# Alexander-H-Liu/End-to-end-ASR-Pytorch

Hardware: NVIDIA H100
Metric: utterances/sec (train step, ~12s@16kHz synthetic) (higher is better)
Workload: dtype f32

## Files before the change

### end-to-end-asr-pytorch_b200/csrc/lstm.cu

```cuda
#include "common.cuh"
#include "lstm_umma.h"
#include "../../include/b200asr.h"
#include "../../include/b200asr_debug.h"

namespace b200asr {

constexpr int LSTM_GTHREADS = 128;
constexpr int LSTM_THREADS = 2 * LSTM_GTHREADS + 64;
constexpr int LSTM_NCHUNK = 4;
constexpr int LSTM_MAX_TILES = 32;
constexpr int LSTM_CHUNK_PAD = 4;
constexpr int LSTM_COUNTER_BYTES = 4096;

struct LstmParams {
    float* gates;
    const float* whh;
    float* cst;
    float* out;
    float* xbuf;
    unsigned* counters;
    int* err_flag;
    int B, T, H, ndir, UB, Bc, nub, nbg, NH, R;
    int b0, Bend;
    int mma;
// ... 1320 lines not shown
extern "C" int b200asr_bilstm_plan(int B, int H, int ndir, int* unit_block, int* batch_block, int* n_ctas) {
    Plan pl;
    const int rc = make_plan(B, H, ndir, &pl);
    B200_REQUIRE(rc == 0, "bilstm_plan: no feasible decomposition for B=%d H=%d ndir=%d (H must be a multiple of 16)",
                 B, H, ndir);
    if (unit_block) *unit_block = pl.UB;
    if (batch_block) *batch_block = pl.Bc;
    if (n_ctas) *n_ctas = pl.ctas;
    return B200_OK;
}

extern "C" int b200asr_bilstm_uses_tensor_cores(int B, int H, int ndir) {
    Plan pl;
    if (make_plan(B, H, ndir, &pl) != 0) return -1;
    return pl.mma ? 1 : 0;
}

static int bilstm_run(bool bwd, float* gates, const float* w_hh, float* cstate, float* out_or_dout, int B, int T,
                      int H, int ndir, void* workspace, size_t workspace_bytes, cudaStream_t stream) {
    B200_REQUIRE(gates && w_hh && cstate && out_or_dout && workspace, "bilstm: null pointer");
    B200_REQUIRE(B > 0 && T > 0 && H > 0 && (ndir == 1 || ndir == 2), "bilstm: bad sizes B=%d T=%d H=%d ndir=%d", B, T,
                 H, ndir);
    Plan pl;
    LstmVariant v;
    B200_REQUIRE(lstm_variant(B, H, ndir, bwd, &pl, &v) == 0,
                 "bilstm: no feasible decomposition for B=%d H=%d ndir=%d (H must be a multiple of 16)", B, H, ndir);
    B200_REQUIRE(workspace_bytes >= b200asr_bilstm_workspace_bytes(B, T, H, ndir), "bilstm: workspace too small");
    if (v.gen == 1 && !bwd)
        return lstm_umma_fwd(gates, w_hh, cstate, out_or_dout, B, T, H, ndir, workspace, workspace_bytes, v.strict != 0,
                             stream);
    if (v.gen == 1)
        return lstm_umma_bwd(gates, w_hh, cstate, out_or_dout, B, T, H, ndir, workspace, workspace_bytes, stream);
    unsigned char* ws = reinterpret_cast<unsigned char*>(workspace);
    float* packed = reinterpret_cast<float*>(ws);
    const size_t xoff = align_up(pl.pack_bytes, 256);
    const size_t xbytes = pl.xbuf_fwd_bytes > pl.xbuf_bwd_bytes ? pl.xbuf_fwd_bytes : pl.xbuf_bwd_bytes;
    float* xbuf = reinterpret_cast<float*>(ws + xoff);
    unsigned* counters = reinterpret_cast<unsigned*>(ws + xoff + align_up(xbytes, 256));
    int* err_flag = reinterpret_cast<int*>(counters + (LSTM_COUNTER_BYTES / 4 - 4));

    {
        const long long n = (long long)(pl.pack_bytes / sizeof(float));
        int blocks = (int)((n + 255) / 256);
        if (blocks > 4096) blocks = 4096;
        if (pl.mma) lstm_pack_mma_kernel<<<blocks, 256, 0, stream>>>(w_hh, packed, H, pl.UB, ndir, bwd ? 1 : 0);
        else lstm_pack_kernel<<<blocks, 256, 0, stream>>>(w_hh, packed, H, pl.UB, ndir, bwd ? 1 : 0);
        B200_LAUNCH_CHECK("lstm_pack_kernel");
    }
    LstmParams p;
    p.gates = gates; p.whh = packed; p.cst = cstate; p.out = out_or_dout; p.xbuf = xbuf; p.counters = counters;
    p.err_flag = err_flag; p.B = B; p.T = T; p.H = H; p.ndir = ndir; p.UB = pl.UB; p.Bc = pl.Bc; p.nub = pl.nub;
    p.nbg = pl.nbg; p.NH = pl.NH; p.R = pl.R; p.mma = pl.mma; p.form = v.form;
    const void* fn = !pl.mma ? (bwd ? (const void*)bilstm_bwd_kernel : (const void*)bilstm_fwd_kernel)
                             : (bwd ? (const void*)bilstm_bwd_mma_kernel : (const void*)bilstm_fwd_mma_kernel);
    const size_t smem = bwd ? pl.smem_bwd : pl.smem_fwd;
    B200_REQUIRE(smem <= (size_t)max_optin_smem(), "bilstm: %zu B of shared memory exceed the device limit", smem);
    B200_CUDA(cudaFuncSetAttribute(fn, cudaFuncAttributeMaxDynamicSharedMemorySize, (int)smem));
    int per_sm = 0;
    B200_CUDA(cudaOccupancyMaxActiveBlocksPerMultiprocessor(&per_sm, fn, LSTM_THREADS, smem));
    B200_REQUIRE((long long)per_sm * sm_count() >= pl.ctas, "bilstm: %d CTAs cannot be co-resident (%d/SM x %d SMs)",
                 pl.ctas, per_sm, sm_count());
    for (int sp = 0; sp < pl.nsplit; ++sp) {
        p.b0 = sp * pl.Bsub;
        p.Bend = p.b0 + pl.Bsub < B ? p.b0 + pl.Bsub : B;
        B200_CUDA(cudaMemsetAsync(counters, 0, LSTM_COUNTER_BYTES, stream));
        void* args[] = {&p};
        B200_CUDA(cudaLaunchCooperativeKernel(fn, dim3(pl.ctas), dim3(LSTM_THREADS), args, smem, stream));
        count_launch();
    }
    return B200_OK;
}

extern "C" int b200asr_debug_lstm_variant(int B, int H, int ndir, int bwd, int* desc) {
    Plan pl;
    LstmVariant v;
    if (B <= 0 || H <= 0 || (ndir != 1 && ndir != 2) || !desc) return -1;
    const int rc = lstm_variant(B, H, ndir, bwd != 0, &pl, &v);
    if (rc != 0) return rc;
    const int d[9] = {v.gen, v.UB, v.UBP, v.poll, v.strict, v.nsplit, v.form, v.R, v.vec};
    for (int i = 0; i < 9; ++i) desc[i] = d[i];
    return 0;
}

extern "C" void b200asr_debug_set_lstm_mode(int mode) {
    g_lstm_mode = mode & 3;
    g_lstm_strict = (mode & 256) != 0;
}

extern "C" int b200asr_bilstm_fwd(float* gates, const float* w_hh, float* cstate, float* out, int B, int T, int H,
                                  int ndir, void* workspace, size_t workspace_bytes, b200asr_stream stream) {
    return bilstm_run(false, gates, w_hh, cstate, out, B, T, H, ndir, workspace, workspace_bytes,
                      (cudaStream_t)stream);
}

extern "C" int b200asr_bilstm_bwd(float* gates, const float* w_hh, const float* cstate, const float* dout, int B,
                                  int T, int H, int ndir, void* workspace, size_t workspace_bytes,
                                  b200asr_stream stream) {
    return bilstm_run(true, gates, w_hh, const_cast<float*>(cstate), const_cast<float*>(dout), B, T, H, ndir,
                      workspace, workspace_bytes, (cudaStream_t)stream);
}

extern "C" int b200asr_lstm_cell_fwd(const float* preact, const float* c_prev, float* gates, float* c, float* h,
                                     int B, int H, b200asr_stream stream) {
    B200_REQUIRE(preact && c_prev && gates && c && h, "lstm_cell_fwd: null pointer");
    B200_REQUIRE(B > 0 && H > 0, "lstm_cell_fwd: bad sizes");
    const int n = B * H;
    lstm_cell_fwd_kernel<<<(n + 255) / 256, 256, 0, (cudaStream_t)stream>>>(preact, c_prev, gates, c, h, B, H);
    B200_LAUNCH_CHECK("lstm_cell_fwd_kernel");
    return B200_OK;
}

extern "C" int b200asr_lstm_cell_bwd(const float* gates, const float* c_prev, const float* c, const float* dh,
                                     const float* dc_next, float* dpreact, float* dc_prev, int B, int H,
                                     b200asr_stream stream) {
    B200_REQUIRE(gates && c_prev && c && dh && dpreact && dc_prev, "lstm_cell_bwd: null pointer");
    B200_REQUIRE(B > 0 && H > 0, "lstm_cell_bwd: bad sizes");
    const int n = B * H;
    lstm_cell_bwd_kernel<<<(n + 255) / 256, 256, 0, (cudaStream_t)stream>>>(gates, c_prev, c, dh, dc_next, dpreact,
                                                                          dc_prev, B, H);
    B200_LAUNCH_CHECK("lstm_cell_bwd_kernel");
    return B200_OK;
}
```

### end-to-end-asr-pytorch_b200/csrc/lstm_umma.cu

```cuda
#include <cuda_fp16.h>
#include "common.cuh"
#include "wgmma.cuh"
#include "lstm_umma.h"

namespace b200asr {
namespace {

constexpr int UL_BC = 32;
constexpr int UL_MAX_CTRL = 8;
constexpr int UL_ATOM_A = 64 * 128;
constexpr int UL_MAX_ATOMS = 16;
constexpr int UL_COUNTER_BYTES = 4096;

struct UlParams {
    float* gates;
    const uint8_t* wpack;
    float* cst;
    float* out;
    uint8_t* xbuf;
    unsigned* counters;
    int* err_flag;
    int B, T, H, ndir, UB, nub, nbg, NA, NC;
    int strict;
    int b0, Bend;
// ... 183 lines not shown
                if (st_pending) {
                    *reinterpret_cast<float4*>(p.gates + (st_row * H + ug) * 4) = st_g;
                    p.cst[st_row * H + ug] = st_c;
                    p.out[st_out] = st_h;
                    st_pending = false;
                }
                const float k = 1.f / 2048.f;
                pre.x += dif[0] + (dif[2] + eif[0]) * k;
                pre.y += dif[1] + (dif[3] + eif[1]) * k;
                pre.z += dgo[0] + (dgo[2] + ego[0]) * k;
                pre.w += dgo[1] + (dgo[3] + ego[1]) * k;
            }
            const float ig = sigmoidf_(pre.x);
            const float fg = sigmoidf_(pre.y);
            const float gg = tanhf(pre.z);
            const float og = sigmoidf_(pre.w);
            const float c = fmaf(fg, c_reg, ig * gg);
            c_reg = ok ? c : 0.f;
            const float hq = ok ? og * tanhf(c) : 0.f;
            if (step + 1 < T) {
                uint8_t* dstimg = xb + (size_t)(step & 1) * img_bytes;
                __half hi, lo;
                split_f16(hq, hi, lo);
                if ((UB & 3) == 0) {
                    uint32_t wh = __half_as_ushort(hi), wl = __half_as_ushort(lo);
                    wh |= __shfl_down_sync(0xffffffffu, wh, 1) << 16;
                    wl |= __shfl_down_sync(0xffffffffu, wl, 1) << 16;
                    const uint32_t wh2 = __shfl_down_sync(0xffffffffu, wh, 2);
                    const uint32_t wl2 = __shfl_down_sync(0xffffffffu, wl, 2);
                    if (tq == 0 && unit < UB) {
                        *reinterpret_cast<uint2*>(dstimg + pub_hi) = make_uint2(wh, wh2);
                        *reinterpret_cast<uint2*>(dstimg + pub_lo) = make_uint2(wl, wl2);
                    }
                } else if (unit < UB) {
                    *reinterpret_cast<__half*>(dstimg + pub_hi) = hi;
                    *reinterpret_cast<__half*>(dstimg + pub_lo) = lo;
                }
                __syncwarp();
                if (lane == 0) ul_arrive(pub);
            }
            st_g = make_float4(ig, fg, gg, og);
            st_c = c;
            st_h = hq;
            st_row = rowbase;
            st_out = ((size_t)brow * T + tt) * (p.ndir * H) + (size_t)dir * H + ug;
            st_pending = ok;
        }
        if (st_pending) {
            *reinterpret_cast<float4*>(p.gates + (st_row * H + ug) * 4) = st_g;
            p.cst[st_row * H + ug] = st_c;
            p.out[st_out] = st_h;
        }
    }
}

template <int UB>
__global__ void ul_pack_bwd_kernel(const float* __restrict__ w, uint8_t* __restrict__ dst, int H, int ndir) {
    const int nub = H / UB;
    const long long per_cta = (long long)2 * H * 64;
    const long long n_el = (long long)ndir * nub * per_cta;
    for (long long i = (long long)blockIdx.x * blockDim.x + threadIdx.x; i < n_el; i += (long long)gridDim.x * blockDim.x) {
        const int cta = (int)(i / per_cta);
        int r = (int)(i - (long long)cta * per_cta);
        const int part = r / (H * 64);
        r -= part * H * 64;
        const int n = r >> 6, k = r & 63;
        const int dir = cta / nub, ub = cta - dir * nub;
        const int u = k >> 2, g = k & 3;
        float v = 0.f;
        if (u < UB) v = w[((long long)dir * 4 * H + (long long)g * H + (ub * UB + u)) * H + n];
        __half hi, lo;
        split_f16(v, hi, lo);
        uint8_t* img = dst + (size_t)cta * ((size_t)2 * H * 128) + (size_t)part * H * 128;
        *reinterpret_cast<__half*>(img + wgmma::sw128_offset(n, k * 2)) = part ? lo : hi;
    }
}


__device__ __forceinline__ float add_ftz(float a, float b) {
    float r;
    asm("add.ftz.f32 %0, %1, %2;" : "=f"(r) : "f"(a), "f"(b));
    return r;
}

constexpr int ULB_EPI_WARPS = 16;
constexpr int ULB_CTRL = 4;

template <int UB>
__global__ void __launch_bounds__(32 * (ULB_EPI_WARPS + 1 + ULB_CTRL), 1) bilstm_bwd_umma_kernel(UlParams p) {
    constexpr int KS = (4 * UB) / 16;
    extern __shared__ __align__(1024) uint8_t smem[];
    const int H = p.H, T = p.T, nub = p.nub;
    const int NB = (H + 255) / 256;
    uint8_t* sWhi = smem;
    uint8_t* sWlo = smem + (size_t)H * 128;
    uint8_t* sA1 = sWlo + (size_t)H * 128;
    uint8_t* sA2 = sA1 + 8192;
    float* rscale = reinterpret_cast<float*>(sA2 + 8192);
    uint64_t* a_ready = reinterpret_cast<uint64_t*>(rscale + 32);
    uint64_t* mma_done = a_ready + 1;
    uint64_t* wload = a_ready + 2;

    const int tid = threadIdx.x, warp = tid >> 5, lane = tid & 31;
    int blk = blockIdx.x;
    const int ub = blk % p.nub; blk /= p.nub;
    const int bg = blk % p.nbg; blk /= p.nbg;
    const int dir = blk;

    for (int i = tid; i < 16384 / 16; i += blockDim.x) reinterpret_cast<uint4*>(sA1)[i] = make_uint4(0, 0, 0, 0);
    if (tid == 0) {
        mbar_init(a_ready, ULB_EPI_WARPS);
        mbar_init(mma_done, ULB_EPI_WARPS);
        mbar_init(wload, 1);
        mbar_fence_init();
    }
    fence_proxy_async_smem();
    __syncthreads();
    const size_t xelems = (size_t)nub * nub * UL_BC * UB;
    float* xb = reinterpret_cast<float*>(p.xbuf) + ((size_t)dir * p.nbg + bg) * 2 * xelems;

    if (warp >= ULB_EPI_WARPS) {
        if (warp == ULB_EPI_WARPS + 1 && lane == 0) {
            const uint8_t* wsrc = p.wpack + ((size_t)dir * p.nub + ub) * ((size_t)2 * H * 128);
            mbar_expect_tx(wload, (uint32_t)(2 * H * 128));
            for (int off = 0; off < 2 * H * 128; off += 32768)
                bulk_g2s(sWhi + off, wsrc + off, 32768, wload);
        }
    } else {
        const int ci = warp * 32 + lane;
        const bool cell = ci < UL_BC * UB;
        const int b = cell ? ci / UB : 0, u = cell ? ci % UB : 0;
        const int brow = p.b0 + bg * UL_BC + b;
        const bool ok = cell && brow < p.Bend;
        const int ug = ub * UB + u;
        const int row_hi = 16 * (b >> 3) + (b & 7), row_lo = row_hi + 8;
        const uint32_t off_hi = wgmma::sw128_offset(row_hi, 8 * u), off_lo = wgmma::sw128_offset(row_lo, 8 * u);
        const int q = warp & 3, jq = warp >> 2, r = lane >> 2, tq = lane & 3;
        const int drow = 8 * q + r;
        const uint32_t a1 = smem_u32(sA1), a2 = smem_u32(sA2), whi = smem_u32(sWhi), wlo = smem_u32(sWlo);
        float d[32];
        float dc_reg = 0.f;

        for (int step = 0; step < T; ++step) {
            const int fstep = T - 1 - step;
            const int tt = dir ? (T - 1 - fstep) : fstep;
            const int tt_prev = dir ? tt + 1 : tt - 1;
            float4 gtv = make_float4(0.f, 0.f, 0.f, 0.f);
            float ct = 0.f, cp = 0.f, dh = 0.f;
            const size_t row = ((size_t)dir * p.B + (ok ? brow : 0)) * T + tt;
            if (ok) {
                gtv = *reinterpret_cast<const float4*>(p.gates + (row * H + ug) * 4);
                ct = p.cst[row * H + ug];
                if (fstep > 0) cp = p.cst[(((size_t)dir * p.B + brow) * T + tt_prev) * H + ug];
                dh = p.out[((size_t)brow * T + tt) * (p.ndir * H) + (size_t)dir * H + ug];
            }
            if (step > 0) {
                if (cell) {
                    const float* ib = xb + (size_t)((step - 1) & 1) * xelems + (size_t)ub * nub * UL_BC * UB +
                                      (size_t)b * UB + u;
                    const uint32_t tag = (uint32_t)(((step - 1) >> 1) & 1) ^ 1u;
                    const long long t0 = clock64();
                    float s0 = 0.f, s1 = 0.f, s2 = 0.f, s3 = 0.f;
                    for (int sb = 0; sb < nub; sb += 32) {
                        float v[32];
                        const int nhere = min(32, nub - sb);
                        v[0] = ld_relaxed_f32(ib + (size_t)sb * UL_BC * UB);
                        while ((__float_as_uint(v[0]) & 1u) != tag) {
                            ul_watchdog(t0, p.err_flag);
                            v[0] = ld_relaxed_f32(ib + (size_t)sb * UL_BC * UB);
                        }
#pragma unroll
                        for (int j = 1; j < 32; ++j)
                            v[j] = (j < nhere) ? ld_relaxed_f32(ib + (size_t)(sb + j) * UL_BC * UB) : __uint_as_float(tag);
                        uint32_t pending = 0;
#pragma unroll
                        for (int j = 1; j < 32; ++j) pending |= ((__float_as_uint(v[j]) & 1u) != tag) ? (1u << j) : 0u;
                        while (pending) {
                            ul_watchdog(t0, p.err_flag);
#pragma unroll
                            for (int j = 1; j < 32; ++j)
                                if (pending & (1u << j)) {
                                    v[j] = ld_relaxed_f32(ib + (size_t)(sb + j) * UL_BC * UB);
                                    if ((__float_as_uint(v[j]) & 1u) == tag) pending &= ~(1u << j);
                                }
                        }
#pragma unroll
                        for (int j = 0; j < 32; j += 4) {
                            if (j < nhere) {
                                s0 = add_ftz(s0, v[j]); s1 = add_ftz(s1, v[j + 1]);
                                s2 = add_ftz(s2, v[j + 2]); s3 = add_ftz(s3, v[j + 3]);
                            }
                        }
                    }
                    dh += (s0 + s1) + (s2 + s3);
                }
            }
            float4 dg = make_float4(0.f, 0.f, 0.f, 0.f);
            if (ok) {
                const float ig = gtv.x, fg = gtv.y, gg = gtv.z, og = gtv.w;
                const float tc = tanhf(ct);
                const float dc = dc_reg + dh * og * (1.f - tc * tc);
                dg.x = dc * gg * ig * (1.f - ig);
                dg.y = dc * cp * fg * (1.f - fg);
                dg.z = dc * ig * (1.f - gg * gg);
                dg.w = dh * tc * og * (1.f - og);
                dc_reg = dc * fg;
                *reinterpret_cast<float4*>(p.gates + (row * H + ug) * 4) = dg;
            }
            if (step + 1 < T) {
                float m = fmaxf(fmaxf(fabsf(dg.x), fabsf(dg.y)), fmaxf(fabsf(dg.z), fabsf(dg.w)));
#pragma unroll
                for (int o = 1; o < UB; o <<= 1) m = fmaxf(m, __shfl_xor_sync(0xffffffffu, m, o));
                int e = (int)((__float_as_uint(m) >> 23) & 0xffu) - 127;
                e = e < -113 ? -113 : (e > 127 ? 127 : e);
                const float sc = __uint_as_float((uint32_t)(127 + 13 - e) << 23);
                if (step > 0) mbar_wait(mma_done, (uint32_t)((step - 1) & 1));
                if (cell) {
                    if (u == 0) rscale[b] = __uint_as_float((uint32_t)(127 + e - 13) << 23);
                    __half hi[4], lo[4];
                    split_f16(dg.x * sc, hi[0], lo[0]);
                    split_f16(dg.y * sc, hi[1], lo[1]);
                    split_f16(dg.z * sc, hi[2], lo[2]);
                    split_f16(dg.w * sc, hi[3], lo[3]);
                    const uint2 vh = make_uint2((uint32_t)__half_as_ushort(hi[0]) | ((uint32_t)__half_as_ushort(hi[1]) << 16),
                                                (uint32_t)__half_as_ushort(hi[2]) | ((uint32_t)__half_as_ushort(hi[3]) << 16));
                    const uint2 vl = make_uint2((uint32_t)__half_as_ushort(lo[0]) | ((uint32_t)__half_as_ushort(lo[1]) << 16),
                                                (uint32_t)__half_as_ushort(lo[2]) | ((uint32_t)__half_as_ushort(lo[3]) << 16));
                    *reinterpret_cast<uint2*>(sA1 + off_hi) = vh;
                    *reinterpret_cast<uint2*>(sA1 + off_lo) = vl;
                    *reinterpret_cast<uint2*>(sA2 + off_lo) = vh;
                }
                fence_proxy_async_smem();
                __syncwarp();
                if (lane == 0) ul_arrive(a_ready);
                if (step == 0) mbar_wait(wload, 0);
                mbar_wait(a_ready, (uint32_t)(step & 1));
                float* outbase = xb + (size_t)(step & 1) * xelems;
                for (int j = 0; j < NB; ++j) {
                    if (256 * j + 64 * jq >= H) continue;
                    const uint32_t boff = (uint32_t)(256 * j + 64 * jq) * 128u;
                    wgmma::fence_operand(d);
                    wgmma::fence();
#pragma unroll
                    for (int kk = 0; kk < KS; ++kk) {
                        wgmma::mma_f16_n64(d, wgmma::desc_k_sw128(a1 + kk * 32), wgmma::desc_k_sw128(whi + boff + kk * 32), kk > 0);
                        wgmma::mma_f16_n64(d, wgmma::desc_k_sw128(a2 + kk * 32), wgmma::desc_k_sw128(wlo + boff + kk * 32), 1);
                    }
                    wgmma::commit_group();
                    wgmma::wait_all();
                    wgmma::fence_operand(d);
                    const float* v0 = d;
                    const float* v1 = d + 16;
                    const float rs = rscale[drow];
                    const float k = 1.f / 2048.f;
#pragma unroll
                    for (int hh = 0; hh < 2; ++hh) {
#pragma unroll
                        for (int g = 0; g < 4; ++g) {
                            const float* v = hh ? &v1[4 * g] : &v0[4 * g];
                            const int n = 256 * j + 64 * jq + 32 * hh + 8 * g + 2 * tq;
                            const int dst = n / UB, uu = n - dst * UB;
                            const float o0 = (v[0] + v[2] * k) * rs;
                            const float o1 = (v[1] + v[3] * k) * rs;
                            float* optr = outbase + (((size_t)dst * nub + ub) * UL_BC + drow) * UB + uu;
                            const uint32_t tagw = (uint32_t)((step >> 1) & 1) ^ 1u;
                            st_relaxed_v2(optr, (__float_as_uint(o0) & ~1u) | tagw, (__float_as_uint(o1) & ~1u) | tagw);
                        }
                    }
                }
                __syncwarp();
                if (lane == 0) ul_arrive(mma_done);
            }
        }
    }
}

struct UlPlan {
    int UB, UBp, nub, nbg, ctas, NA, Bsub, nsplit;
    size_t smem, pack_bytes, xbuf_bytes;
};

int ul_plan(int B, int H, int ndir, UlPlan* out) {
    if (H % 64 != 0 || H / 64 > UL_MAX_ATOMS) return -1;
    const int sms = sm_count();
    const size_t cap = (size_t)max_optin_smem();
    const int NA = H / 64;
    for (int n = 1; n <= B; ++n) {
        const int Bs = (B + n - 1) / n;
        const int nbg = (Bs + UL_BC - 1) / UL_BC;
        for (int UB = 2; UB <= 16; ++UB) {
            if (H % UB) continue;
            const int UBp = (UB + 3) / 4 * 4;
            if (UBp != 8 && UBp != 12 && UBp != 16) continue;
            const int nub = H / UB;
            const int ctas = ndir * nbg * nub;
            if (ctas > sms) continue;
            const size_t smem = (size_t)NA * UL_ATOM_A + (size_t)NA * 8 * UBp * 128 + 512;
            if (smem > cap) continue;
            if ((size_t)ndir * nbg * UL_MAX_ATOMS * 4 > UL_COUNTER_BYTES - 64) continue;
            out->UB = UB; out->UBp = UBp; out->nub = nub; out->nbg = nbg; out->ctas = ctas; out->NA = NA;
            out->Bsub = Bs; out->nsplit = (B + Bs - 1) / Bs; out->smem = smem;
            out->pack_bytes = (size_t)ndir * nub * NA * 8 * UBp * 128;
            out->xbuf_bytes = (size_t)ndir * nbg * 2 * NA * UL_ATOM_A;
            return 0;
        }
        if (Bs <= UL_BC) break;
    }
    return -2;
}

size_t ul_align(size_t x) { return (x + 255) / 256 * 256; }

template <int UBP>
int ul_launch_fwd(const UlPlan& pl, UlParams p, const float* w_hh, cudaStream_t stream) {
    {
        const long long n = (long long)p.ndir * pl.nub * 8 * UBP * p.H;
        int blocks = (int)((n + 255) / 256);
        if (blocks > 8192) blocks = 8192;
        ul_pack_fwd_kernel<UBP><<<blocks, 256, 0, stream>>>(w_hh, const_cast<uint8_t*>(p.wpack), p.H, pl.UB, p.ndir);
        B200_LAUNCH_CHECK("ul_pack_fwd_kernel");
    }
    const void* fn = (const void*)bilstm_fwd_umma_kernel<UBP>;
    B200_CUDA(cudaFuncSetAttribute(fn, cudaFuncAttributeMaxDynamicSharedMemorySize, (int)pl.smem));
    int per_sm = 0;
    const int threads = 32 * (UBP + 1 + p.NC);
    B200_CUDA(cudaOccupancyMaxActiveBlocksPerMultiprocessor(&per_sm, fn, threads, pl.smem));
    B200_REQUIRE((long long)per_sm * sm_count() >= pl.ctas, "bilstm(umma): %d CTAs cannot be co-resident (%d/SM x %d SMs)",
                 pl.ctas, per_sm, sm_count());
    for (int sp = 0; sp < pl.nsplit; ++sp) {
        p.b0 = sp * pl.Bsub;
        p.Bend = p.b0 + pl.Bsub < p.B ? p.b0 + pl.Bsub : p.B;
        B200_CUDA(cudaMemsetAsync(p.counters, 0, UL_COUNTER_BYTES, stream));
        void* args[] = {&p};
        B200_CUDA(cudaLaunchCooperativeKernel(fn, dim3(pl.ctas), dim3(threads), args, pl.smem, stream));
        count_launch();
    }
    return B200_OK;
}

struct UlbPlan {
    int UB, nub, nbg, ctas, Bsub, nsplit;
    size_t smem, pack_bytes, xbuf_bytes;
};

int ulb_plan(int B, int H, int ndir, UlbPlan* out) {
    if (H % 128 != 0 || H < 256 || H > 768) return -1;
    const int sms = sm_count();
    const size_t cap = (size_t)max_optin_smem();
    for (int n = 1; n <= B; ++n) {
        const int Bs = (B + n - 1) / n;
        const int nbg = (Bs + UL_BC - 1) / UL_BC;
        for (int UB = 8; UB <= 16; UB += 8) {
            if (H % UB) continue;
            const int nub = H / UB;
            const int ctas = ndir * nbg * nub;
            if (ctas > sms) continue;
            if (nub % 4) continue;
            const size_t inbox = (size_t)nub * UL_BC * UB * 4;
            const size_t smem = (size_t)2 * H * 128 + 16384 + 128 + 128;
            if (smem > cap || (inbox / ULB_CTRL) % 16 || (2 * H * 128) % 32768) continue;
            out->UB = UB; out->nub = nub; out->nbg = nbg; out->ctas = ctas; out->Bsub = Bs;
            out->nsplit = (B + Bs - 1) / Bs; out->smem = smem;
            out->pack_bytes = (size_t)ndir * nub * 2 * H * 128;
            out->xbuf_bytes = (size_t)ndir * nbg * 2 * nub * inbox;
            return 0;
        }
        if (Bs <= UL_BC) break;
    }
    return -2;
}

template <int UB>
int ul_launch_bwd(const UlbPlan& pl, UlParams p, const float* w_hh, cudaStream_t stream) {
    {
        const long long n = (long long)p.ndir * pl.nub * 2 * p.H * 64;
        int blocks = (int)((n + 255) / 256);
        if (blocks > 8192) blocks = 8192;
        ul_pack_bwd_kernel<UB><<<blocks, 256, 0, stream>>>(w_hh, const_cast<uint8_t*>(p.wpack), p.H, p.ndir);
        B200_LAUNCH_CHECK("ul_pack_bwd_kernel");
    }
    const void* fn = (const void*)bilstm_bwd_umma_kernel<UB>;
    B200_CUDA(cudaFuncSetAttribute(fn, cudaFuncAttributeMaxDynamicSharedMemorySize, (int)pl.smem));
    int per_sm = 0;
    const int threads = 32 * (ULB_EPI_WARPS + 1 + ULB_CTRL);
    B200_CUDA(cudaOccupancyMaxActiveBlocksPerMultiprocessor(&per_sm, fn, threads, pl.smem));
    B200_REQUIRE((long long)per_sm * sm_count() >= pl.ctas, "bilstm(umma bwd): %d CTAs cannot be co-resident (%d/SM x %d SMs)",
                 pl.ctas, per_sm, sm_count());
    for (int sp = 0; sp < pl.nsplit; ++sp) {
        p.b0 = sp * pl.Bsub;
        p.Bend = p.b0 + pl.Bsub < p.B ? p.b0 + pl.Bsub : p.B;
        B200_CUDA(cudaMemsetAsync(p.counters, 0, UL_COUNTER_BYTES, stream));
        B200_CUDA(cudaMemsetAsync(p.xbuf, 0, pl.xbuf_bytes, stream));
        void* args[] = {&p};
        B200_CUDA(cudaLaunchCooperativeKernel(fn, dim3(pl.ctas), dim3(threads), args, pl.smem, stream));
        count_launch();
    }
    return B200_OK;
}

}

bool lstm_umma_bwd_variant(int B, int H, int ndir, int* ub, int* nsplit) {
    UlbPlan pl;
    if (ulb_plan(B, H, ndir, &pl) != 0) return false;
    *ub = pl.UB;
    *nsplit = pl.nsplit;
    return true;
}

bool lstm_umma_fwd_variant(int B, int H, int ndir, int* ub, int* ubp, int* nsplit) {
    UlPlan pl;
    if (ul_plan(B, H, ndir, &pl) != 0) return false;
    *ub = pl.UB;
    *ubp = pl.UBp;
    *nsplit = pl.nsplit;
    return true;
}

int lstm_umma_bwd(float* gates, const float* w_hh, const float* cstate, const float* dout, int B, int T, int H, int ndir,
                  void* workspace, size_t workspace_bytes, cudaStream_t stream) {
    UlbPlan pl;
    B200_REQUIRE(ulb_plan(B, H, ndir, &pl) == 0, "bilstm(umma bwd): unsupported shape B=%d H=%d ndir=%d", B, H, ndir);
    B200_REQUIRE(workspace_bytes >= lstm_umma_workspace_bytes(B, H, ndir), "bilstm(umma bwd): workspace too small");
    uint8_t* ws = reinterpret_cast<uint8_t*>(workspace);
    UlParams p;
    p.gates = gates; p.cst = const_cast<float*>(cstate); p.out = const_cast<float*>(dout);
    p.wpack = ws;
    p.xbuf = ws + ul_align(pl.pack_bytes);
    p.counters = reinterpret_cast<unsigned*>(ws + ul_align(pl.pack_bytes) + ul_align(pl.xbuf_bytes));
    p.err_flag = reinterpret_cast<int*>(p.counters + (UL_COUNTER_BYTES / 4 - 4));
    p.B = B; p.T = T; p.H = H; p.ndir = ndir; p.UB = pl.UB; p.nub = pl.nub; p.nbg = pl.nbg; p.NA = 0; p.NC = ULB_CTRL;
    p.strict = 0;
    p.b0 = 0; p.Bend = B;
    if (pl.UB == 16) return ul_launch_bwd<16>(pl, p, w_hh, stream);
    return ul_launch_bwd<8>(pl, p, w_hh, stream);
}

size_t lstm_umma_workspace_bytes(int B, int H, int ndir) {
    UlPlan pl;
    UlbPlan pb;
    size_t f = 0, b = 0;
    if (ul_plan(B, H, ndir, &pl) == 0) f = ul_align(pl.pack_bytes) + ul_align(pl.xbuf_bytes) + UL_COUNTER_BYTES;
    if (ulb_plan(B, H, ndir, &pb) == 0) b = ul_align(pb.pack_bytes) + ul_align(pb.xbuf_bytes) + UL_COUNTER_BYTES;
    return f > b ? f : b;
}

int lstm_umma_plan(int B, int H, int ndir, int* unit_block, int* batch_block, int* n_ctas) {
    UlPlan pl;
    if (ul_plan(B, H, ndir, &pl) != 0) return -1;
    if (unit_block) *unit_block = pl.UB;
    if (batch_block) *batch_block = UL_BC;
    if (n_ctas) *n_ctas = pl.ctas;
    return 0;
}

int lstm_umma_fwd(float* gates, const float* w_hh, float* cstate, float* out, int B, int T, int H, int ndir,
                  void* workspace, size_t workspace_bytes, bool strict, cudaStream_t stream) {
    UlPlan pl;
    B200_REQUIRE(ul_plan(B, H, ndir, &pl) == 0, "bilstm(umma): unsupported shape B=%d H=%d ndir=%d", B, H, ndir);
    B200_REQUIRE(workspace_bytes >= lstm_umma_workspace_bytes(B, H, ndir), "bilstm(umma): workspace too small");
    uint8_t* ws = reinterpret_cast<uint8_t*>(workspace);
    UlParams p;
    p.gates = gates; p.cst = cstate; p.out = out;
    p.wpack = ws;
    p.xbuf = ws + ul_align(pl.pack_bytes);
    p.counters = reinterpret_cast<unsigned*>(ws + ul_align(pl.pack_bytes) + ul_align(pl.xbuf_bytes));
    p.err_flag = reinterpret_cast<int*>(p.counters + (UL_COUNTER_BYTES / 4 - 4));
    p.B = B; p.T = T; p.H = H; p.ndir = ndir; p.UB = pl.UB; p.nub = pl.nub; p.nbg = pl.nbg; p.NA = pl.NA;
    p.NC = pl.NA < UL_MAX_CTRL ? pl.NA : UL_MAX_CTRL;
    p.strict = strict ? 1 : 0;
    p.b0 = 0; p.Bend = B;
    switch (pl.UBp) {
        case 8: return ul_launch_fwd<8>(pl, p, w_hh, stream);
        case 12: return ul_launch_fwd<12>(pl, p, w_hh, stream);
        default: return ul_launch_fwd<16>(pl, p, w_hh, stream);
    }
}

}
```

### end-to-end-asr-pytorch_b200/csrc/lstm_umma.h

```cpp
#pragma once
#include <cuda_runtime.h>
#include <stddef.h>

namespace b200asr {

bool lstm_umma_fwd_variant(int B, int H, int ndir, int* ub, int* ubp, int* nsplit);
bool lstm_umma_bwd_variant(int B, int H, int ndir, int* ub, int* nsplit);
int lstm_umma_bwd(float* gates, const float* w_hh, const float* cstate, const float* dout, int B, int T, int H, int ndir,
                  void* workspace, size_t workspace_bytes, cudaStream_t stream);
size_t lstm_umma_workspace_bytes(int B, int H, int ndir);
int lstm_umma_plan(int B, int H, int ndir, int* unit_block, int* batch_block, int* n_ctas);
int lstm_umma_fwd(float* gates, const float* w_hh, float* cstate, float* out, int B, int T, int H, int ndir,
                  void* workspace, size_t workspace_bytes, bool strict, cudaStream_t stream);

}
```

### end-to-end-asr-pytorch_b200/lib.py

```python
import ctypes
import os
from ctypes import c_int, c_float, c_double, c_longlong, c_size_t, c_void_p, c_char_p, c_ulonglong, POINTER

import torch

_HERE = os.path.dirname(os.path.abspath(__file__))
LIB_PATH = os.path.join(_HERE, "libb200asr.so")

_lib = None

_P = c_void_p
SIGNATURES = {
    "b200asr_version": (c_int, []),
    "b200asr_last_error": (c_char_p, []),
    "b200asr_launch_count": (c_ulonglong, []),
    "b200asr_launch_count_reset": (None, []),
    "b200asr_device_sm_count": (c_int, []),
    "b200asr_fbank_fwd": (c_int, [_P, _P, c_int, c_int, c_int, c_int, c_int, c_float, c_int, _P, c_int, _P, _P, _P, _P,
                                  c_int, c_int, c_float, _P, c_int, _P, _P]),
    "b200asr_fbank_fwd_pcm16": (c_int, [_P, _P, c_int, c_int, c_int, c_int, c_int, c_float, c_int, _P, c_int, _P, _P, _P, _P,
                                  c_int, c_int, c_float, _P, c_int, _P, _P]),
    "b200asr_delta_cmvn_workspace_bytes": (c_size_t, [c_int, c_int, c_int, c_int]),
    "b200asr_delta_cmvn_fwd": (c_int, [_P, _P, c_int, c_int, c_int, c_int, c_int, c_int, c_float, _P, _P, c_size_t,
                                       _P]),
    "b200asr_log_softmax_fwd": (c_int, [_P, _P, _P, _P, c_longlong, c_int, _P]),
    "b200asr_log_softmax_bwd": (c_int, [_P, _P, _P, c_longlong, c_int, _P]),
    "b200asr_ctc_workspace_bytes": (c_size_t, [c_int, c_int, c_int]),
    "b200asr_ctc_fwd_bwd": (c_int, [_P, c_longlong, c_longlong, _P, _P, _P, c_int, c_int, c_int, c_int, c_int, _P, _P,
                                    _P, _P, c_size_t, _P]),
    "b200asr_ctc_grad": (c_int, [_P, c_longlong, c_longlong, _P, _P, _P, c_int, c_int, c_int, c_int, c_int, _P, _P, _P,
                                 _P, _P, c_size_t, _P]),
    "b200asr_ctc_fwd_bwd_logits": (c_int, [_P, _P, c_longlong, c_longlong, _P, _P, _P, c_int, c_int, c_int, c_int, c_int, _P,
                                           _P, _P, _P, c_size_t, _P]),
    "b200asr_ctc_grad_logits": (c_int, [_P, _P, c_longlong, c_longlong, _P, _P, _P, c_int, c_int, c_int, c_int, c_int, _P,
                                        _P, _P, _P, _P, c_size_t, _P]),
    "b200asr_ctc_prefix_score": (c_int, [_P, c_int, c_int, _P, _P, _P, _P, c_int, c_int, c_int, c_int, _P, _P, _P]),
    "b200asr_bilstm_workspace_bytes": (c_size_t, [c_int, c_int, c_int, c_int]),
    "b200asr_bilstm_plan": (c_int, [c_int, c_int, c_int, POINTER(c_int), POINTER(c_int), POINTER(c_int)]),
    "b200asr_bilstm_uses_tensor_cores": (c_int, [c_int, c_int, c_int]),
    "b200asr_bilstm_uses_tcgen05": (c_int, [c_int, c_int, c_int]),
    "b200asr_bilstm_fwd": (c_int, [_P, _P, _P, _P, c_int, c_int, c_int, c_int, _P, c_size_t, _P]),
    "b200asr_bilstm_bwd": (c_int, [_P, _P, _P, _P, c_int, c_int, c_int, c_int, _P, c_size_t, _P]),
    "b200asr_debug_set_lstm_mode": (None, [c_int]),
    "b200asr_debug_lstm_variant": (c_int, [c_int, c_int, c_int, c_int, POINTER(c_int)]),
    "b200asr_debug_ctc_variant": (c_int, [c_int]),
    "b200asr_debug_locattn_bwd_minb": (c_int, [c_int, c_int, c_int, c_int]),
    "b200asr_debug_dotattn_bwd_minb": (c_int, [c_int, c_int, c_int]),
    "b200asr_debug_locattn_heads_bwd_minb": (c_int, [c_int, c_int, c_int, c_int, c_int]),
    "b200asr_debug_gemm_plan": (c_int, [c_int, c_int, c_int, c_int, c_int, c_size_t, POINTER(c_int)]),
    "b200asr_lstm_cell_fwd": (c_int, [_P, _P, _P, _P, _P, c_int, c_int, _P]),
    "b200asr_lstm_cell_bwd": (c_int, [_P, _P, _P, _P, _P, _P, _P, c_int, c_int, _P]),
    "b200asr_gru_cell_fwd": (c_int, [_P, _P, _P, _P, c_int, c_int, _P]),
    "b200asr_gru_cell_bwd": (c_int, [_P, _P, _P, _P, _P, c_int, c_int, _P]),
    "b200asr_locattn_cluster_size": (c_int, [c_int, c_int]),
    "b200asr_locattn_wpart_floats": (c_size_t, [c_int, c_int, c_int]),
    "b200asr_locattn_fwd": (c_int, [_P, _P, _P, _P, _P, _P, _P, _P, _P, c_float, c_int, c_int, c_int, c_int, c_int,
                                    c_int, _P, _P, _P]),
    "b200asr_locattn_bwd": (c_int, [_P, _P, _P, _P, _P, _P, _P, _P, c_float, _P, _P, _P, c_int, c_int, c_int, c_int,
                                    c_int, c_int, _P, _P, _P, _P, _P, _P]),
    "b200asr_locattn_bwd_acc": (c_int, [_P, _P, _P, _P, _P, _P, _P, _P, c_float, _P, _P, _P, c_int, c_int, c_int, c_int,
                                        c_int, c_int, _P, _P, _P, _P, _P]),
    "b200asr_attn_dvalue": (c_int, [_P, _P, c_int, c_int, c_int, c_int, _P, c_int, _P]),
    "b200asr_dotattn_supported": (c_int, [c_int, c_int, c_int]),
    "b200asr_dotattn_fwd": (c_int, [_P, _P, _P, _P, c_int, c_float, c_int, c_int, c_int, c_int, _P, _P, _P]),
    "b200asr_dotattn_bwd_acc": (c_int, [_P, _P, _P, _P, c_int, c_float, _P, _P, _P, c_int, c_int, c_int, c_int, _P, _P,
                                        _P]),
    "b200asr_locattn_heads_supported": (c_int, [c_int, c_int, c_int, c_int, c_int, c_int]),
    "b200asr_locattn_heads_wpart_floats": (c_size_t, [c_int, c_int, c_int, c_int]),
    "b200asr_locattn_heads_fwd": (c_int, [_P, _P, _P, _P, _P, _P, _P, _P, _P, c_float, c_int, c_int, c_int, c_int, c_int,
                                          c_int, c_int, _P, _P, _P]),
    "b200asr_locattn_heads_bwd_acc": (c_int, [_P, _P, _P, _P, _P, _P, _P, _P, c_float, _P, _P, _P, c_int, c_int, c_int,
                                              c_int, c_int, c_int, c_int, _P, _P, _P, _P, _P]),
    "b200asr_ce_fwd_bwd": (c_int, [_P, _P, c_longlong, c_longlong, c_int, _P, _P, _P, _P]),
    "b200asr_embedding_bwd_workspace_bytes": (c_size_t, [c_int, c_int]),
    "b200asr_embedding_bwd": (c_int, [_P, _P, c_int, c_int, c_int, _P, _P, c_size_t, _P]),
    "b200asr_gemm3x_tn": (c_int, [_P, c_int, _P, _P, _P, _P, c_int, c_int, c_int, c_int, c_int, _P, c_size_t, _P]),
    "b200asr_gemm3x_nn": (c_int, [_P, c_int, _P, c_int, _P, _P, c_int, c_int, c_int, c_int, c_int, _P, c_size_t, _P]),
    "b200asr_gemm3x_workspace_bytes": (c_size_t, [c_int, c_int]),
    "b200asr_gemm3x_nt": (c_int, [_P, c_longlong, c_longlong, c_int, _P, c_longlong, c_longlong, c_int, _P, c_int, c_int,
                                  c_int, c_int, c_int, c_int, c_int, _P, c_size_t, _P]),
    "b200asr_tf32_residual": (c_int, [_P, _P, c_longlong, _P]),
    "b200asr_conv3x3_fwd": (c_int, [_P, c_int, c_int, _P, _P, _P, c_int, _P, c_int, c_int, c_int, c_int, _P]),
    "b200asr_conv3x3_wgrad": (c_int, [_P, _P, c_int, c_int, _P, c_int, c_int, c_int, c_int, _P, c_size_t, _P]),
    "b200asr_vgg_im2col": (c_int, [_P, c_longlong, c_int, c_int, c_int, c_int, _P, _P]),
    "b200asr_vgg_pool_fwd": (c_int, [_P, c_int, c_int, c_int, c_int, _P, _P, c_int, _P]),
    "b200asr_vgg_pool_bwd": (c_int, [_P, _P, _P, c_int, c_int, c_int, c_int, _P, c_int, _P]),
    "b200asr_vgg_feat_grad": (c_int, [_P, _P, c_int, c_int, c_int, c_int, c_int, c_int, _P, _P]),
    "b200asr_f16x3_padded_k": (c_int, [c_int]),
    "b200asr_f16x3_split_rows": (c_int, [_P, c_longlong, c_int, c_int, _P, _P, _P, _P]),
    "b200asr_f16x3_split_cols": (c_int, [_P, c_longlong, c_longlong, c_int, c_int, c_int, c_int, _P, _P, _P, _P]),
    "b200asr_f16x3_split_dg": (c_int, [_P, c_int, c_int, c_int, _P, _P, _P, _P, _P, _P, _P, _P]),
    "b200asr_gemm_f16x3": (c_int, [_P, _P, _P, _P, _P, _P, _P, _P, c_int, c_int, c_int, c_int, c_int, c_int, _P, c_size_t,
                                   _P]),
    "b200asr_split_tf32": (c_int, [_P, _P, _P, c_longlong, _P]),
    "b200asr_grad_norm_scratch_bytes": (c_size_t, []),
    "b200asr_grad_norm": (c_int, [_P, c_longlong, _P, _P, _P]),
    "b200asr_adadelta_step": (c_int, [_P, _P, _P, _P, c_longlong, c_float, c_double, c_float, c_float, _P, c_float, _P,
                                      _P]),
    "b200asr_adam_step": (c_int, [_P, _P, _P, _P, c_longlong, c_float, c_double, c_double, c_float, c_float, _P,
                                  c_float, _P, _P]),
}


class B200AsrError(RuntimeError):
    pass


def load(build_if_missing=False):
    global _lib
    if _lib is not None:
        return _lib
    if not os.path.exists(LIB_PATH):
        if build_if_missing:
            from . import _build
            _build.build()
        else:
            raise B200AsrError(
                "libb200asr.so is missing (%s): run `python -c 'import __graft_entry__ as g; g.build()'`; "
                "there is no CPU fallback" % LIB_PATH)
    lib = ctypes.CDLL(LIB_PATH)
    for name, (res, args) in SIGNATURES.items():
        fn = getattr(lib, name)
        fn.restype = res
        fn.argtypes = args
    _lib = lib
    return lib

# ... 69 lines not shown
```

### include/b200asr_debug.h

```cpp
#ifndef B200ASR_DEBUG_H
#define B200ASR_DEBUG_H
#include "b200asr.h"
#ifdef __cplusplus
extern "C" {
#endif

B200ASR_API void b200asr_debug_set_lstm_mode(int mode);
B200ASR_API int b200asr_debug_lstm_variant(int B, int H, int ndir, int bwd, int* desc);
B200ASR_API int b200asr_debug_ctc_variant(int L_max);
B200ASR_API int b200asr_debug_locattn_bwd_minb(int B, int T, int D, int E);
B200ASR_API int b200asr_debug_dotattn_bwd_minb(int R, int T, int E);
B200ASR_API int b200asr_debug_locattn_heads_bwd_minb(int B, int N, int T, int D, int E);
B200ASR_API int b200asr_debug_gemm_plan(int form, int M, int N, int K, int batches, size_t workspace_bytes, int* desc);

#ifdef __cplusplus
}
#endif
#endif
```

Before: 837.3.

## Pre-reduce LSTM backward partial sums across thread-block clusters via distributed shared memory

The backward recurrent LSTM kernel gains a thread-block-cluster variant. Each CTA sends its per-step partial hidden-gradient contributions to a peer CTA's shared memory using mapa and cluster-scoped stores. The owning CTA sums them, then publishes one aggregated slice to the global exchange buffer. This cuts the number of global sources each CTA must poll and sum per timestep by the cluster size, and shrinks the exchange buffer. The cost is extra shared-memory staging, an intra-cluster spin-wait per step, and a cooperative-plus-cluster launch that falls back to the non-cluster kernel if the launch is refused.

```diff
diff --git a/end-to-end-asr-pytorch_b200/csrc/lstm.cu b/end-to-end-asr-pytorch_b200/csrc/lstm.cu
--- a/end-to-end-asr-pytorch_b200/csrc/lstm.cu
+++ b/end-to-end-asr-pytorch_b200/csrc/lstm.cu
@@ -1426,9 +1426,19 @@
     return 0;
 }
 
+extern "C" int b200asr_debug_lstm_cluster(int B, int H, int ndir, int bwd) {
+    Plan pl;
+    LstmVariant v;
+    if (B <= 0 || H <= 0 || (ndir != 1 && ndir != 2)) return -1;
+    const int rc = lstm_variant(B, H, ndir, bwd != 0, &pl, &v);
+    if (rc != 0) return rc;
+    return (bwd && v.gen == 1) ? lstm_umma_bwd_cluster(B, H, ndir) : 1;
+}
+
 extern "C" void b200asr_debug_set_lstm_mode(int mode) {
     g_lstm_mode = mode & 3;
     g_lstm_strict = (mode & 256) != 0;
+    lstm_umma_set_cluster_cap((mode >> 4) & 7);
 }
 
 extern "C" int b200asr_bilstm_fwd(float* gates, const float* w_hh, float* cstate, float* out, int B, int T, int H,
diff --git a/end-to-end-asr-pytorch_b200/csrc/lstm_umma.cu b/end-to-end-asr-pytorch_b200/csrc/lstm_umma.cu
--- a/end-to-end-asr-pytorch_b200/csrc/lstm_umma.cu
+++ b/end-to-end-asr-pytorch_b200/csrc/lstm_umma.cu
@@ -289,13 +289,35 @@
     asm("add.ftz.f32 %0, %1, %2;" : "=f"(r) : "f"(a), "f"(b));
     return r;
 }
+__device__ __forceinline__ uint32_t mapa_shared(uint32_t addr, int rank) {
+    uint32_t r;
+    asm volatile("mapa.shared::cluster.u32 %0, %1, %2;" : "=r"(r) : "r"(addr), "r"(rank));
+    return r;
+}
+__device__ __forceinline__ void st_cluster_v2(uint32_t addr, uint32_t a, uint32_t b) {
+    asm volatile("st.relaxed.cluster.shared::cluster.v2.u32 [%0], {%1,%2};" ::"r"(addr), "r"(a), "r"(b) : "memory");
+}
+__device__ __forceinline__ uint2 ld_cluster_v2(uint32_t addr) {
+    uint2 v;
+    asm volatile("ld.relaxed.cluster.shared::cta.v2.u32 {%0,%1}, [%2];" : "=r"(v.x), "=r"(v.y) : "r"(addr) : "memory");
+    return v;
+}
+__device__ __forceinline__ void cluster_sync_all() {
+    asm volatile("barrier.cluster.arrive.release;\n\tbarrier.cluster.wait.acquire;" ::: "memory");
+}
 
 constexpr int ULB_EPI_WARPS = 16;
 constexpr int ULB_CTRL = 4;
-
-template <int UB>
+constexpr size_t ULB_SMEM_FIXED = 16384 + 128 + 128;
+
+__host__ __device__ inline size_t ulb_staging_bytes(int nub, int UB, int CS) {
+    return CS > 1 ? (size_t)2 * (CS - 1) * (nub / CS) * UL_BC * UB * 4 : 0;
+}
+
+template <int UB, int CS>
 __global__ void __launch_bounds__(32 * (ULB_EPI_WARPS + 1 + ULB_CTRL), 1) bilstm_bwd_umma_kernel(UlParams p) {
     constexpr int KS = (4 * UB) / 16;
+    static_assert(64 % (UB * CS) == 0, "cluster size");
     extern __shared__ __align__(1024) uint8_t smem[];
     const int H = p.H, T = p.T, nub = p.nub;
     const int NB = (H + 255) / 256;
@@ -307,14 +329,22 @@
     uint64_t* a_ready = reinterpret_cast<uint64_t*>(rscale + 32);
     uint64_t* mma_done = a_ready + 1;
     uint64_t* wload = a_ready + 2;
+    float* stg = reinterpret_cast<float*>(sA1 + ULB_SMEM_FIXED);
 
     const int tid = threadIdx.x, warp = tid >> 5, lane = tid & 31;
     int blk = blockIdx.x;
     const int ub = blk % p.nub; blk /= p.nub;
     const int bg = blk % p.nbg; blk /= p.nbg;
     const int dir = blk;
+    const int crank = ub % CS;
+    const int nsrc = nub / CS;
+    constexpr int PB = 32 / CS;
 
     for (int i = tid; i < 16384 / 16; i += blockDim.x) reinterpret_cast<uint4*>(sA1)[i] = make_uint4(0, 0, 0, 0);
+    if (CS > 1) {
+        for (int i = tid; i < (int)(ulb_staging_bytes(nub, UB, CS) / 16); i += blockDim.x)
+            reinterpret_cast<uint4*>(stg)[i] = make_uint4(0, 0, 0, 0);
+    }
     if (tid == 0) {
         mbar_init(a_ready, ULB_EPI_WARPS);
         mbar_init(mma_done, ULB_EPI_WARPS);
@@ -322,9 +352,11 @@
         mbar_fence_init();
     }
     fence_proxy_async_smem();
-    __syncthreads();
-    const size_t xelems = (size_t)nub * nub * UL_BC * UB;
+    if (CS > 1) cluster_sync_all();
+    else __syncthreads();
+    const size_t xelems = (size_t)nub * nsrc * UL_BC * UB;
     float* xb = reinterpret_cast<float*>(p.xbuf) + ((size_t)dir * p.nbg + bg) * 2 * xelems;
+    const uint32_t stg_base = smem_u32(stg), stg_slot = (uint32_t)nsrc * (UL_BC * UB * 4);
 
     if (warp >= ULB_EPI_WARPS) {
         if (warp == ULB_EPI_WARPS + 1 && lane == 0) {
@@ -363,36 +395,36 @@
             }
             if (step > 0) {
                 if (cell) {
-                    const float* ib = xb + (size_t)((step - 1) & 1) * xelems + (size_t)ub * nub * UL_BC * UB +
+                    const float* ib = xb + (size_t)((step - 1) & 1) * xelems + (size_t)ub * nsrc * UL_BC * UB +
                                       (size_t)b * UB + u;
                     const uint32_t tag = (uint32_t)(((step - 1) >> 1) & 1) ^ 1u;
                     const long long t0 = clock64();
                     float s0 = 0.f, s1 = 0.f, s2 = 0.f, s3 = 0.f;
-                    for (int sb = 0; sb < nub; sb += 32) {
-                        float v[32];
-                        const int nhere = min(32, nub - sb);
+                    for (int sb = 0; sb < nsrc; sb += PB) {
+                        float v[PB];
+                        const int nhere = min(PB, nsrc - sb);
                         v[0] = ld_relaxed_f32(ib + (size_t)sb * UL_BC * UB);
                         while ((__float_as_uint(v[0]) & 1u) != tag) {
                             ul_watchdog(t0, p.err_flag);
                             v[0] = ld_relaxed_f32(ib + (size_t)sb * UL_BC * UB);
                         }
 #pragma unroll
-                        for (int j = 1; j < 32; ++j)
+                        for (int j = 1; j < PB; ++j)
                             v[j] = (j < nhere) ? ld_relaxed_f32(ib + (size_t)(sb + j) * UL_BC * UB) : __uint_as_float(tag);
                         uint32_t pending = 0;
 #pragma unroll
-                        for (int j = 1; j < 32; ++j) pending |= ((__float_as_uint(v[j]) & 1u) != tag) ? (1u << j) : 0u;
+                        for (int j = 1; j < PB; ++j) pending |= ((__float_as_uint(v[j]) & 1u) != tag) ? (1u << j) : 0u;
                         while (pending) {
                             ul_watchdog(t0, p.err_flag);
 #pragma unroll
-                            for (int j = 1; j < 32; ++j)
+                            for (int j = 1; j < PB; ++j)
                                 if (pending & (1u << j)) {
                                     v[j] = ld_relaxed_f32(ib + (size_t)(sb + j) * UL_BC * UB);
                                     if ((__float_as_uint(v[j]) & 1u) == tag) pending &= ~(1u << j);
                                 }
                         }
 #pragma unroll
-                        for (int j = 0; j < 32; j += 4) {
+                        for (int j = 0; j < PB; j += 4) {
                             if (j < nhere) {
                                 s0 = add_ftz(s0, v[j]); s1 = add_ftz(s1, v[j + 1]);
                                 s2 = add_ftz(s2, v[j + 2]); s3 = add_ftz(s3, v[j + 3]);
@@ -460,18 +492,65 @@
                     const float* v1 = d + 16;
                     const float rs = rscale[drow];
                     const float k = 1.f / 2048.f;
+                    const uint32_t tagw = (uint32_t)((step >> 1) & 1) ^ 1u;
+                    constexpr int G = UB / 8;
+                    float own[16 / CS];
 #pragma unroll
                     for (int hh = 0; hh < 2; ++hh) {
 #pragma unroll
                         for (int g = 0; g < 4; ++g) {
                             const float* v = hh ? &v1[4 * g] : &v0[4 * g];
-                            const int n = 256 * j + 64 * jq + 32 * hh + 8 * g + 2 * tq;
+                            const int m = 4 * hh + g;
+                            const int n = 256 * j + 64 * jq + 8 * m + 2 * tq;
                             const int dst = n / UB, uu = n - dst * UB;
+                            const int agg = (8 * m / UB) % CS;
                             const float o0 = (v[0] + v[2] * k) * rs;
                             const float o1 = (v[1] + v[3] * k) * rs;
-                            float* optr = outbase + (((size_t)dst * nub + ub) * UL_BC + drow) * UB + uu;
-                            const uint32_t tagw = (uint32_t)((step >> 1) & 1) ^ 1u;
-                            st_relaxed_v2(optr, (__float_as_uint(o0) & ~1u) | tagw, (__float_as_uint(o1) & ~1u) | tagw);
+                            if (CS > 1 && agg == crank) {
+                                const int idx = (m / G) / CS * G + m % G;
+                                own[2 * idx] = o0;
+                                own[2 * idx + 1] = o1;
+                                continue;
+                            }
+                            const uint32_t w0 = (__float_as_uint(o0) & ~1u) | tagw, w1 = (__float_as_uint(o1) & ~1u) | tagw;
+                            if (CS == 1) {
+                                st_relaxed_v2(outbase + (((size_t)dst * nsrc + ub) * UL_BC + drow) * UB + uu, w0, w1);
+                            } else {
+                                const int slot = (crank - agg - 1 + CS) % CS;
+                                const uint32_t sa = stg_base + (uint32_t)((step & 1) * (CS - 1) + slot) * stg_slot +
+                                                    (uint32_t)(((dst / CS) * UL_BC + drow) * UB + uu) * 4u;
+                                st_cluster_v2(mapa_shared(sa, agg), w0, w1);
+                            }
+                        }
+                    }
+                    if (CS > 1) {
+                        const long long t0 = clock64();
+#pragma unroll
+                        for (int idx = 0; idx < 8 / CS; ++idx) {
+                            const int m = G * (crank + CS * (idx / G)) + idx % G;
+                            const int n = 256 * j + 64 * jq + 8 * m + 2 * tq;
+                            const int dst = n / UB, uu = n - dst * UB;
+                            const uint32_t soff = (uint32_t)(((dst / CS) * UL_BC + drow) * UB + uu) * 4u;
+                            float s0 = 0.f, s1 = 0.f;
+#pragma unroll
+                            for (int rr = 0; rr < CS; ++rr) {
+                                float x0 = own[2 * idx], x1 = own[2 * idx + 1];
+                                if (rr != crank) {
+                                    const int slot = (rr - crank - 1 + CS) % CS;
+                                    const uint32_t sa = stg_base + (uint32_t)((step & 1) * (CS - 1) + slot) * stg_slot + soff;
+                                    uint2 w = ld_cluster_v2(sa);
+                                    while (((w.x & 1u) != tagw) || ((w.y & 1u) != tagw)) {
+                                        ul_watchdog(t0, p.err_flag);
+                                        w = ld_cluster_v2(sa);
+                                    }
+                                    x0 = __uint_as_float(w.x);
+                                    x1 = __uint_as_float(w.y);
+                                }
+                                s0 = add_ftz(s0, x0);
+                                s1 = add_ftz(s1, x1);
+                            }
+                            st_relaxed_v2(outbase + (((size_t)dst * nsrc + ub / CS) * UL_BC + drow) * UB + uu,
+                                          (__float_as_uint(s0) & ~1u) | tagw, (__float_as_uint(s1) & ~1u) | tagw);
                         }
                     }
                 }
@@ -480,6 +559,7 @@
             }
         }
     }
+    if (CS > 1) cluster_sync_all();
 }
 
 struct UlPlan {
@@ -547,10 +627,70 @@
 
 struct UlbPlan {
     int UB, nub, nbg, ctas, Bsub, nsplit;
+    int CS;
     size_t smem, pack_bytes, xbuf_bytes;
 };
 
-int ulb_plan(int B, int H, int ndir, UlbPlan* out) {
+int g_ulb_cs_cap = 0;
+bool g_ulb_coop_refused = false;
+
+const void* ulb_kernel(int UB, int CS) {
+    if (UB == 16)
+        return CS == 4 ? (const void*)bilstm_bwd_umma_kernel<16, 4>
+                       : CS == 2 ? (const void*)bilstm_bwd_umma_kernel<16, 2> : (const void*)bilstm_bwd_umma_kernel<16, 1>;
+    return CS == 4 ? (const void*)bilstm_bwd_umma_kernel<8, 4>
+                   : CS == 2 ? (const void*)bilstm_bwd_umma_kernel<8, 2> : (const void*)bilstm_bwd_umma_kernel<8, 1>;
+}
+
+void ulb_launch_config(cudaLaunchConfig_t* cfg, cudaLaunchAttribute* attr, int ctas, int CS, size_t smem,
+                       cudaStream_t stream) {
+    *cfg = cudaLaunchConfig_t{};
+    cfg->gridDim = dim3(ctas);
+    cfg->blockDim = dim3(32 * (ULB_EPI_WARPS + 1 + ULB_CTRL));
+    cfg->dynamicSmemBytes = smem;
+    cfg->stream = stream;
+    attr[0].id = cudaLaunchAttributeCooperative;
+    attr[0].val.cooperative = 1;
+    attr[1].id = cudaLaunchAttributeClusterDimension;
+    attr[1].val.clusterDim.x = CS;
+    attr[1].val.clusterDim.y = 1;
+    attr[1].val.clusterDim.z = 1;
+    cfg->attrs = attr;
+    cfg->numAttrs = 2;
+}
+
+int ulb_max_clusters(int UB, int CS, int ctas, size_t smem) {
+    const void* fn = ulb_kernel(UB, CS);
+    if (cudaFuncSetAttribute(fn, cudaFuncAttributeMaxDynamicSharedMemorySize, (int)smem) != cudaSuccess) {
+        (void)cudaGetLastError();
+        return 0;
+    }
+    cudaLaunchConfig_t cfg;
+    cudaLaunchAttribute attr[2];
+    ulb_launch_config(&cfg, attr, ctas, CS, smem, 0);
+    cfg.attrs = attr + 1;
+    cfg.numAttrs = 1;
+    int n = 0;
+    if (cudaOccupancyMaxActiveClusters(&n, fn, &cfg) != cudaSuccess) {
+        (void)cudaGetLastError();
+        return 0;
+    }
+    return n;
+}
+
+int ulb_cluster(const UlbPlan& pl, size_t cap) {
+    for (int cs = 4; cs >= 2; cs >>= 1) {
+        if (g_ulb_coop_refused || (g_ulb_cs_cap != 0 && cs > g_ulb_cs_cap)) continue;
+        if (pl.nub % cs || (pl.nub / cs) % 4) continue;
+        const size_t smem = pl.smem + ulb_staging_bytes(pl.nub, pl.UB, cs);
+        if (smem > cap) continue;
+        if ((long long)ulb_max_clusters(pl.UB, cs, pl.ctas, smem) * cs < pl.ctas) continue;
+        return cs;
+    }
+    return 1;
+}
+
+int ulb_plan(int B, int H, int ndir, UlbPlan* out, bool cluster = true) {
     if (H % 128 != 0 || H < 256 || H > 768) return -1;
     const int sms = sm_count();
     const size_t cap = (size_t)max_optin_smem();
@@ -564,12 +704,14 @@
             if (ctas > sms) continue;
             if (nub % 4) continue;
             const size_t inbox = (size_t)nub * UL_BC * UB * 4;
-            const size_t smem = (size_t)2 * H * 128 + 16384 + 128 + 128;
+            const size_t smem = (size_t)2 * H * 128 + ULB_SMEM_FIXED;
             if (smem > cap || (inbox / ULB_CTRL) % 16 || (2 * H * 128) % 32768) continue;
             out->UB = UB; out->nub = nub; out->nbg = nbg; out->ctas = ctas; out->Bsub = Bs;
             out->nsplit = (B + Bs - 1) / Bs; out->smem = smem;
             out->pack_bytes = (size_t)ndir * nub * 2 * H * 128;
             out->xbuf_bytes = (size_t)ndir * nbg * 2 * nub * inbox;
+            out->CS = cluster ? ulb_cluster(*out, cap) : 1;
+            out->smem += ulb_staging_bytes(nub, UB, out->CS);
             return 0;
         }
         if (Bs <= UL_BC) break;
@@ -578,7 +720,7 @@
 }
 
 template <int UB>
-int ul_launch_bwd(const UlbPlan& pl, UlParams p, const float* w_hh, cudaStream_t stream) {
+int ul_launch_bwd(UlbPlan pl, UlParams p, const float* w_hh, cudaStream_t stream) {
     {
         const long long n = (long long)p.ndir * pl.nub * 2 * p.H * 64;
         int blocks = (int)((n + 255) / 256);
@@ -586,34 +728,58 @@
         ul_pack_bwd_kernel<UB><<<blocks, 256, 0, stream>>>(w_hh, const_cast<uint8_t*>(p.wpack), p.H, p.ndir);
         B200_LAUNCH_CHECK("ul_pack_bwd_kernel");
     }
-    const void* fn = (const void*)bilstm_bwd_umma_kernel<UB>;
-    B200_CUDA(cudaFuncSetAttribute(fn, cudaFuncAttributeMaxDynamicSharedMemorySize, (int)pl.smem));
-    int per_sm = 0;
-    const int threads = 32 * (ULB_EPI_WARPS + 1 + ULB_CTRL);
-    B200_CUDA(cudaOccupancyMaxActiveBlocksPerMultiprocessor(&per_sm, fn, threads, pl.smem));
-    B200_REQUIRE((long long)per_sm * sm_count() >= pl.ctas, "bilstm(umma bwd): %d CTAs cannot be co-resident (%d/SM x %d SMs)",
-                 pl.ctas, per_sm, sm_count());
-    for (int sp = 0; sp < pl.nsplit; ++sp) {
-        p.b0 = sp * pl.Bsub;
-        p.Bend = p.b0 + pl.Bsub < p.B ? p.b0 + pl.Bsub : p.B;
-        B200_CUDA(cudaMemsetAsync(p.counters, 0, UL_COUNTER_BYTES, stream));
-        B200_CUDA(cudaMemsetAsync(p.xbuf, 0, pl.xbuf_bytes, stream));
-        void* args[] = {&p};
-        B200_CUDA(cudaLaunchCooperativeKernel(fn, dim3(pl.ctas), dim3(threads), args, pl.smem, stream));
-        count_launch();
-    }
-    return B200_OK;
+    for (;;) {
+        const void* fn = ulb_kernel(UB, pl.CS);
+        B200_CUDA(cudaFuncSetAttribute(fn, cudaFuncAttributeMaxDynamicSharedMemorySize, (int)pl.smem));
+        if (pl.CS == 1) {
+            int per_sm = 0;
+            B200_CUDA(cudaOccupancyMaxActiveBlocksPerMultiprocessor(&per_sm, fn, 32 * (ULB_EPI_WARPS + 1 + ULB_CTRL),
+                                                                    pl.smem));
+            B200_REQUIRE((long long)per_sm * sm_count() >= pl.ctas,
+                         "bilstm(umma bwd): %d CTAs cannot be co-resident (%d/SM x %d SMs)", pl.ctas, per_sm, sm_count());
+        }
+        cudaLaunchConfig_t cfg;
+        cudaLaunchAttribute attr[2];
+        ulb_launch_config(&cfg, attr, pl.ctas, pl.CS, pl.smem, stream);
+        bool refused = false;
+        for (int sp = 0; sp < pl.nsplit; ++sp) {
+            p.b0 = sp * pl.Bsub;
+            p.Bend = p.b0 + pl.Bsub < p.B ? p.b0 + pl.Bsub : p.B;
+            B200_CUDA(cudaMemsetAsync(p.counters, 0, UL_COUNTER_BYTES, stream));
+            B200_CUDA(cudaMemsetAsync(p.xbuf, 0, pl.xbuf_bytes, stream));
+            void* args[] = {&p};
+            const cudaError_t e = cudaLaunchKernelExC(&cfg, fn, args);
+            if (e != cudaSuccess && pl.CS > 1 && sp == 0) {
+                (void)cudaGetLastError();
+                refused = true;
+                break;
+            }
+            B200_CUDA(e);
+            count_launch();
+        }
+        if (!refused) return B200_OK;
+        g_ulb_coop_refused = true;
+        pl.smem -= ulb_staging_bytes(pl.nub, UB, pl.CS);
+        pl.CS = 1;
+    }
 }
 
 }
 
 bool lstm_umma_bwd_variant(int B, int H, int ndir, int* ub, int* nsplit) {
     UlbPlan pl;
-    if (ulb_plan(B, H, ndir, &pl) != 0) return false;
+    if (ulb_plan(B, H, ndir, &pl, false) != 0) return false;
     *ub = pl.UB;
     *nsplit = pl.nsplit;
     return true;
 }
+
+int lstm_umma_bwd_cluster(int B, int H, int ndir) {
+    UlbPlan pl;
+    return ulb_plan(B, H, ndir, &pl) == 0 ? pl.CS : -1;
+}
+
+void lstm_umma_set_cluster_cap(int cap) { g_ulb_cs_cap = cap; }
 
 bool lstm_umma_fwd_variant(int B, int H, int ndir, int* ub, int* ubp, int* nsplit) {
     UlPlan pl;
@@ -648,7 +814,7 @@
     UlbPlan pb;
     size_t f = 0, b = 0;
     if (ul_plan(B, H, ndir, &pl) == 0) f = ul_align(pl.pack_bytes) + ul_align(pl.xbuf_bytes) + UL_COUNTER_BYTES;
-    if (ulb_plan(B, H, ndir, &pb) == 0) b = ul_align(pb.pack_bytes) + ul_align(pb.xbuf_bytes) + UL_COUNTER_BYTES;
+    if (ulb_plan(B, H, ndir, &pb, false) == 0) b = ul_align(pb.pack_bytes) + ul_align(pb.xbuf_bytes) + UL_COUNTER_BYTES;
     return f > b ? f : b;
 }
 
diff --git a/end-to-end-asr-pytorch_b200/csrc/lstm_umma.h b/end-to-end-asr-pytorch_b200/csrc/lstm_umma.h
--- a/end-to-end-asr-pytorch_b200/csrc/lstm_umma.h
+++ b/end-to-end-asr-pytorch_b200/csrc/lstm_umma.h
@@ -6,6 +6,8 @@
 
 bool lstm_umma_fwd_variant(int B, int H, int ndir, int* ub, int* ubp, int* nsplit);
 bool lstm_umma_bwd_variant(int B, int H, int ndir, int* ub, int* nsplit);
+int lstm_umma_bwd_cluster(int B, int H, int ndir);
+void lstm_umma_set_cluster_cap(int cap);
 int lstm_umma_bwd(float* gates, const float* w_hh, const float* cstate, const float* dout, int B, int T, int H, int ndir,
                   void* workspace, size_t workspace_bytes, cudaStream_t stream);
 size_t lstm_umma_workspace_bytes(int B, int H, int ndir);
diff --git a/end-to-end-asr-pytorch_b200/lib.py b/end-to-end-asr-pytorch_b200/lib.py
--- a/end-to-end-asr-pytorch_b200/lib.py
+++ b/end-to-end-asr-pytorch_b200/lib.py
@@ -43,6 +43,7 @@
     "b200asr_bilstm_bwd": (c_int, [_P, _P, _P, _P, c_int, c_int, c_int, c_int, _P, c_size_t, _P]),
     "b200asr_debug_set_lstm_mode": (None, [c_int]),
     "b200asr_debug_lstm_variant": (c_int, [c_int, c_int, c_int, c_int, POINTER(c_int)]),
+    "b200asr_debug_lstm_cluster": (c_int, [c_int, c_int, c_int, c_int]),
     "b200asr_debug_ctc_variant": (c_int, [c_int]),
     "b200asr_debug_locattn_bwd_minb": (c_int, [c_int, c_int, c_int, c_int]),
     "b200asr_debug_dotattn_bwd_minb": (c_int, [c_int, c_int, c_int]),
diff --git a/include/b200asr_debug.h b/include/b200asr_debug.h
--- a/include/b200asr_debug.h
+++ b/include/b200asr_debug.h
@@ -6,6 +6,7 @@
 #endif
 
 B200ASR_API void b200asr_debug_set_lstm_mode(int mode);
+B200ASR_API int b200asr_debug_lstm_cluster(int B, int H, int ndir, int bwd);
 B200ASR_API int b200asr_debug_lstm_variant(int B, int H, int ndir, int bwd, int* desc);
 B200ASR_API int b200asr_debug_ctc_variant(int L_max);
 B200ASR_API int b200asr_debug_locattn_bwd_minb(int B, int T, int D, int E);
```

After: 874.6, median of 6. 1.04x the previous value.
